# zhing2006/hala-renderer

Hardware: AMD Instinct MI355X
Metric: Mrays/s (higher is better)
Workload: dtype f32

## Files before the change

### hala-renderer_amd/csrc/trace_shadow.hip

```cpp
#include "trace_loop.h"
#include "variants.h"

namespace rt {
template <bool COUNT, bool STAGED, bool ALPHA, bool INST, bool GROUPS>
__global__ void __launch_bounds__(kTraverseThreads, STAGED ? kTraverseWavesPerSimdStaged : kTraverseWavesPerSimd)
k_trace_shadow(SceneView sv, Queues q, PathState ps, Control* __restrict__ ctl, uint32_t depth, uint32_t kind, uint2* __restrict__ spill_base,
               uint32_t refill) {
  const TraverseLds lds = stage_bvh<STAGED, INST>(sv, g_smem);
  const uint32_t n = ctl->sizes.n_shadow[kind][depth];
  uint2* spill = lane_spill(spill_base);
  StepCounters sc;
  auto src = shadow_source<ALPHA, GROUPS>(q, ps, kind);
  persistent_trace<true, COUNT, STAGED, ALPHA, INST>(sv, lds, spill, &ctl->work_shadow[kind], n, refill, src, sc);
  if (COUNT) flush_counters(ctl, 1, sc);
}

template <bool STAGED, bool ALPHA, bool INST, bool GROUPS>
__global__ void __launch_bounds__(kTraverseThreads, STAGED ? kTraverseWavesPerSimdStaged : kTraverseWavesPerSimd)
k_trace_shadow_then_batch(SceneView sv, const Tri* __restrict__ tris_any, Queues q, PathState ps, Control* __restrict__ ctl, uint32_t depth,
                          uint32_t kinds, const hala_ray* __restrict__ rays, hala_hit* __restrict__ hits, uint2* __restrict__ spill_base, uint32_t refill) {
  const TraverseLds lds = stage_bvh<STAGED, INST>(sv, g_smem);
  uint2* spill = lane_spill(spill_base);
  StepCounters sc;
  {
    SceneView sva = sv;
    sva.tris = tris_any;
    for (uint32_t kind = 0; kind < 2u; ++kind) {
      if (!((kinds >> kind) & 1u)) continue;
      auto src = shadow_source<ALPHA, GROUPS>(q, ps, kind);
      persistent_trace<true, false, STAGED, ALPHA, INST>(sva, lds, spill, &ctl->work_shadow[kind], ctl->sizes.n_shadow[kind][depth], refill, src, sc);
    }
  }
  if (rays == nullptr) return;
  const uint32_t n = ctl->sizes.n_active[depth + 1u];
  if (blockIdx.x == 0 && threadIdx.x == 0) ctl->totals.rays_closest += n;
  BatchSource src{rays, hits, false, true, STAGED && refill == 64u};
  persistent_trace<false, false, STAGED, false, INST>(sv, lds, spill, &ctl->work_closest, n, refill, src, sc);
}
uint32_t trace_shadow_blocks_per_cu(size_t dynamic_lds_bytes, TreeForm tree) {
  return tree_blocks_per_cu([](auto STAGED, auto INST) { return k_trace_shadow<false, STAGED, false, INST, false>; }, tree, kTraverseThreads, dynamic_lds_bytes);
}

void launch_trace_shadow(const LaunchCfg& lc, const SceneView& sv0, const Queues& q, const PathState& ps, Control* ctl, uint32_t depth,
                         uint32_t kind, bool count, hipStream_t s) {
  SceneView sv = sv0;
  sv.tris = sv0.tris_any;
  const TreeForm tree = tree_form(sv);
  dispatch<kFamilyTraceShadow>([&](auto COUNT, auto ALPHA, auto STAGED, auto INST, auto GROUPS) {
    hipLaunchKernelGGL((k_trace_shadow<COUNT, STAGED, ALPHA, INST, GROUPS>), dim3(lc.persistent_blocks), dim3(kTraverseThreads), lc.smem, s, sv, q, ps,
                       ctl, depth, kind, lc.spill, lc.refill);
  }, count, sv.any_translucent != 0u, tree == TreeForm::Staged, tree == TreeForm::TwoLevel, kind == 0u && ps.groups != nullptr);
}

bool launch_trace_shadow_then_batch(const LaunchCfg& lc, const SceneView& sv, const Queues& q, const PathState& ps, Control* ctl, uint32_t depth,
                                    uint32_t kinds, bool with_closest, hipStream_t s) {
  const TreeForm tree = tree_form(sv);
  if (tree == TreeForm::Staged && sv.tris_any != sv.tris) return false;
  const hala_ray* rays = with_closest ? q.rays[(depth + 1u) & 1u] : nullptr;
  dispatch<kFamilyTraceShadowThenBatch>([&](auto ALPHA, auto STAGED, auto INST, auto GROUPS) {
    hipLaunchKernelGGL((k_trace_shadow_then_batch<STAGED, ALPHA, INST, GROUPS>), dim3(lc.persistent_blocks), dim3(kTraverseThreads), lc.smem, s, sv,
                       sv.tris_any, q, ps, ctl, depth, kinds, rays, q.hits, lc.spill, lc.refill);
  }, sv.any_translucent != 0u, tree == TreeForm::Staged, tree == TreeForm::TwoLevel, (kinds & 1u) != 0u && ps.groups != nullptr);
  return true;
}

}
```

Baseline: 6204.

## Assign fused-kernel blocks to closest/light/env roles by cost-weighted ray counts

In the fused shadow-then-closest persistent kernel, each group of 16 blocks now gets a starting role: closest-hit, light shadow, or env shadow. Roles are proportioned by the queue sizes weighted by per-ray cost constants. Blocks start on their assigned queue and then move on to the remaining work, instead of every block draining the shadow queues first and the closest queue last. The aim is to spread contention on the work counters and reduce the tail imbalance between phases. The cost constants are tuned empirically, and the role computation adds a small float calculation per block.

After: 6362 (median of 6 runs). 1.03x the previous value.

```diff
diff --git a/hala-renderer_amd/csrc/trace_shadow.hip b/hala-renderer_amd/csrc/trace_shadow.hip
--- a/hala-renderer_amd/csrc/trace_shadow.hip
+++ b/hala-renderer_amd/csrc/trace_shadow.hip
@@ -15,6 +15,30 @@
   if (COUNT) flush_counters(ctl, 1, sc);
 }
 
+#ifndef RT_FUSED_ROLES
+#define RT_FUSED_ROLES 3
+#endif
+#ifndef RT_ROLE_COST_CLOSEST
+#define RT_ROLE_COST_CLOSEST 153.0f
+#endif
+#ifndef RT_ROLE_COST_ANY
+#define RT_ROLE_COST_ANY 129.0f
+#endif
+constexpr uint32_t kRoleGroup = 16;
+RT_DI uint32_t fused_role(uint32_t n_light, uint32_t n_env, uint32_t n_closest) {
+  const float wl = (float)n_light * RT_ROLE_COST_ANY, we = (float)n_env * RT_ROLE_COST_ANY, wc = (float)n_closest * RT_ROLE_COST_CLOSEST;
+  const float wa = wl + we;
+  if (!(wa + wc > 0.0f)) return 0u;
+  const uint32_t g = blockIdx.x / kRoleGroup;
+  const float fc = wc / (wa + wc);
+  const uint32_t c0 = (uint32_t)((float)g * fc + 0.5f), c1 = (uint32_t)((float)(g + 1u) * fc + 0.5f);
+  if (c1 != c0) return 2u;
+  if (RT_FUSED_ROLES == 2 || !(wa > 0.0f)) return 0u;
+  const uint32_t a = g - c0;
+  const float fl = wl / wa;
+  return (uint32_t)((float)(a + 1u) * fl + 0.5f) != (uint32_t)((float)a * fl + 0.5f) ? 0u : 1u;
+}
+
 template <bool STAGED, bool ALPHA, bool INST, bool GROUPS>
 __global__ void __launch_bounds__(kTraverseThreads, STAGED ? kTraverseWavesPerSimdStaged : kTraverseWavesPerSimd)
 k_trace_shadow_then_batch(SceneView sv, const Tri* __restrict__ tris_any, Queues q, PathState ps, Control* __restrict__ ctl, uint32_t depth,
@@ -22,6 +46,29 @@
   const TraverseLds lds = stage_bvh<STAGED, INST>(sv, g_smem);
   uint2* spill = lane_spill(spill_base);
   StepCounters sc;
+#if RT_FUSED_ROLES
+  const uint32_t n_light = (kinds & 1u) ? ctl->sizes.n_shadow[0][depth] : 0u, n_env = (kinds & 2u) ? ctl->sizes.n_shadow[1][depth] : 0u;
+  const uint32_t n_closest = rays != nullptr ? ctl->sizes.n_active[depth + 1u] : 0u;
+  const uint32_t role = lane0_u32(fused_role(n_light, n_env, n_closest));
+  auto closest = [&]() {
+    const uint32_t n = ctl->sizes.n_active[depth + 1u];
+    if (blockIdx.x == 0 && threadIdx.x == 0) ctl->totals.rays_closest += n;
+    BatchSource src{rays, hits, false, true, STAGED && refill == 64u};
+    persistent_trace<false, false, STAGED, false, INST>(sv, lds, spill, &ctl->work_closest, n, refill, src, sc);
+  };
+  if (role == 2u) closest();
+  {
+    SceneView sva = sv;
+    sva.tris = tris_any;
+    for (uint32_t i = 0; i < 2u; ++i) {
+      const uint32_t kind = i ^ (role & 1u);
+      if (!((kinds >> kind) & 1u)) continue;
+      auto src = shadow_source<ALPHA, GROUPS>(q, ps, kind);
+      persistent_trace<true, false, STAGED, ALPHA, INST>(sva, lds, spill, &ctl->work_shadow[kind], ctl->sizes.n_shadow[kind][depth], refill, src, sc);
+    }
+  }
+  if (role != 2u && rays != nullptr) closest();
+#else
   {
     SceneView sva = sv;
     sva.tris = tris_any;
@@ -36,6 +83,7 @@
   if (blockIdx.x == 0 && threadIdx.x == 0) ctl->totals.rays_closest += n;
   BatchSource src{rays, hits, false, true, STAGED && refill == 64u};
   persistent_trace<false, false, STAGED, false, INST>(sv, lds, spill, &ctl->work_closest, n, refill, src, sc);
+#endif
 }
 uint32_t trace_shadow_blocks_per_cu(size_t dynamic_lds_bytes, TreeForm tree) {
   return tree_blocks_per_cu([](auto STAGED, auto INST) { return k_trace_shadow<false, STAGED, false, INST, false>; }, tree, kTraverseThreads, dynamic_lds_bytes);
```
